# baurst/liso

Measured on AMD Instinct MI355X. Metric: LISO train-step frames/sec (120k-pt clouds), higher is better.
Workload: dtype bf16 (detector, BASELINE configs[2]) + f32 via bf16x3 MFMA (SLIM); north_star's 1e-3 on logits / flow is met by `parity_leg` (f32 via bf16x3 MFMA everywhere) and `fp32_exact_leg`, not by the bf16 detector

## Files before the change

### include/liso_flow_cluster.h

```cpp
#ifndef LISO_FLOW_CLUSTER_H
#define LISO_FLOW_CLUSTER_H

#include <stddef.h>
#include <stdint.h>

#ifdef __cplusplus
extern "C" {
#endif

size_t liso_bev_dynamic_flow_workspace_bytes(int batch, int h, int w);

int liso_bev_dynamic_flow_f32(const float* points, int point_stride, const uint8_t* valid, const int32_t* pillar_coors,
                              const float* flow, int flow_stride, const double* odom_minus_eye, int batch, int n, int h,
                              int w, float* dynamicness, float* nonrigid_flow, void* workspace, size_t workspace_bytes,
                              void* stream);

int liso_odom_inverse_minus_eye_f64(const double* odom, int batch, double* out, void* stream);

size_t liso_fit_box_z_workspace_bytes(int n_points, int n_boxes);

int liso_fit_box_z_f32(const float* points, int point_stride, int n, const float* box_pos, int pos_dims,
                       const float* box_dims, int dims_dims, const float* box_rot, int k, float box_height,
                       int64_t* num_pts, float* fitted_z, float* fitted_height, void* workspace, size_t workspace_bytes,
                       void* stream);

// ... 1 lines not shown
    int batch, gx, gy;
    int window;
    int min_samples;
    float eps;
    float flow_weight;
} liso_dbscan_cfg;

int liso_dbscan_components(const liso_dbscan_cfg* cfg, const uint8_t* dynamic_mask, const float* row_coords,
                           const float* col_coords, const float* flow, uint8_t* core, int32_t* parent, int32_t* is_root,
                           void* stream);

int liso_dbscan_labels(const liso_dbscan_cfg* cfg, const uint8_t* dynamic_mask, const float* row_coords, const float* col_coords,
                       const float* flow, const uint8_t* core, const int32_t* parent, const int32_t* root_rank,
                       int32_t* labels, void* stream);

int liso_region_props(const int32_t* labels, int batch, int gx, int gy, int max_labels, uint64_t* moments, double* props,
                      void* stream);

size_t liso_region_props_workspace_bytes(int batch, int gx, int gy, int max_labels);
int liso_region_props_ws(const int32_t* labels, int batch, int gx, int gy, int max_labels, uint64_t* moments, double* props,
                         void* workspace, size_t workspace_bytes, void* stream);

#ifdef __cplusplus
}
#endif
#endif
```

### liso_amd/_lib.py

```python
import ctypes
import os

import torch

_HERE = os.path.dirname(os.path.abspath(__file__))
LIB_PATH = os.path.join(_HERE, "libliso_hip.so")

_lib = None


class LisoHipError(RuntimeError):
    pass


_ERRORS = {-1: "LISO_EINVAL (bad pointer/size)", -2: "LISO_EWORKSPACE (workspace too small)",
           -3: "LISO_ELAUNCH (HIP launch failed)", -4: "LISO_GROUND_ELENGTH (int(67 / delta_R) > 255)"}


def _preload_torch_hip_runtime():
    tl = os.path.join(os.path.dirname(torch.__file__), "lib", "libamdhip64.so")
    if os.path.exists(tl):
        ctypes.CDLL(tl, mode=ctypes.RTLD_GLOBAL)


# ... 105 lines not shown
    "liso_pfn_forward_rows": (_i, [_vp, _vp, _vp, _vp, _i, _vp, _vp, _vp, _vp, _i, _i, _vp, _vp, _vp]),
    "liso_pfn_backward": (_i, [_vp, _vp, _vp, _vp, _i, _vp, _vp, _vp, _vp, _vp, _i, _vp, _i, _vp, _vp, _vp, _vp, _vp]),
    "liso_pfn_bn_prepare_sub_f32": (_i, [_vp, _vp, _vp, _i, _i, _vp, _vp, _vp, _vp, _vp, _vp, _f, _f, _i, _vp, _vp, _vp, _vp]),
    "liso_pfn_forward_scatter_sub": (_i, [_vp, _vp, _vp, _vp, _i, _i, _vp, _vp, _vp, _vp, _i, _vp, _vp]),
    "liso_pfn_forward_rows_sub": (_i, [_vp, _vp, _vp, _vp, _i, _i, _vp, _vp, _vp, _vp, _i, _i, _vp, _vp, _vp]),
    "liso_pfn_backward_sub": (_i, [_vp, _vp, _vp, _vp, _i, _i, _vp, _vp, _vp, _vp, _vp, _i, _vp, _i, _vp, _vp, _vp, _vp, _vp]),
    "liso_kabsch_workspace_bytes": (_sz, [_vp]),
    "liso_kabsch_trafos_f32": (_i, [_vp, _vp, _vp, _vp, _vp, _vp, _vp, _vp, _vp, _vp, _vp, _sz, _vp]),
    "liso_kabsch_trafos_counted_f32": (_i, [_vp, _vp, _vp, _vp, _vp, _vp, _vp, _vp, _vp, _vp, _vp, _vp, _sz, _vp]),
    "liso_symm_ortho_fwd_f64": (_i, [_vp, _i, _vp, _vp, _vp, _vp, _vp]),
    "liso_symm_ortho_bwd_f64": (_i, [_vp, _vp, _vp, _vp, _i, _vp, _vp]),
    "liso_weighted_moments_workspace_bytes": (_sz, [_i]),
    "liso_weighted_moments_fwd_f32": (_i, [_vp, _vp, _vp, _i, ctypes.c_long, _vp, _vp, _sz, _vp]),
    "liso_weighted_moments_bwd_f32": (_i, [_vp, _vp, _vp, _i, ctypes.c_long, _vp, _vp, _vp, _vp, _vp]),
    "liso_bev_dynamic_flow_workspace_bytes": (_sz, [_i, _i, _i]),
    "liso_bev_dynamic_flow_f32": (_i, [_vp, _i, _vp, _vp, _vp, _i, _vp, _i, _i, _i, _i, _vp, _vp, _vp, _sz, _vp]),
    "liso_odom_inverse_minus_eye_f64": (_i, [_vp, _i, _vp, _vp]),
    "liso_fit_box_z_workspace_bytes": (_sz, [_i, _i]),
    "liso_fit_box_z_f32": (_i, [_vp, _i, _i, _vp, _i, _vp, _i, _vp, _i, _f, _vp, _vp, _vp, _vp, _sz, _vp]),
    "liso_dbscan_components": (_i, [_vp, _vp, _vp, _vp, _vp, _vp, _vp, _vp, _vp]),
    "liso_dbscan_labels": (_i, [_vp, _vp, _vp, _vp, _vp, _vp, _vp, _vp, _vp, _vp]),
    "liso_region_props": (_i, [_vp, _i, _i, _i, _i, _vp, _vp, _vp]),
    "liso_region_props_workspace_bytes": (_sz, [_i, _i, _i, _i]),
    "liso_region_props_ws": (_i, [_vp, _i, _i, _i, _i, _vp, _vp, _vp, _sz, _vp]),
    "liso_corr_lookup_fwd_f32": (_i, [_vp, _vp, _vp, _vp, _vp, _vp]),
    "liso_corr_lookup_fwd_tiled_f32": (_i, [_vp, _vp, _vp, _vp, _vp, _vp]),
    "liso_corr_lookup_bwd_dvol_f32": (_i, [_vp, _vp, _vp, _vp, _vp]),
    "liso_corr_pyramid_fwd_f32": (_i, [_vp, _vp, _vp, _vp]),
    "liso_corr_pyramid_bwd_f32": (_i, [_vp, _vp, _vp, _vp]),
    "liso_corr_bwd_features_workspace_bytes": (_sz, [_vp]),
    "liso_corr_bwd_features_f32": (_i, [_vp, _i, _vp, _vp, _vp, _vp, _vp, _vp, _sz, _vp]),
    "liso_rows_combine_f32": (_i, [_lg, _i, _vp, _lg, _vp, _lg, _vp, _lg, _vp, _lg, _vp, _lg, _i, _vp]),
    "liso_gru_out_rows_train_f32": (_i, [_lg, _i, _vp, _lg, _vp, _vp, _lg, _vp, _lg, _vp]),
    "liso_gru_out_rows_bwd_f32": (_i, [_lg, _i, _vp, _lg, _vp, _vp, _lg, _vp, _lg, _vp, _lg, _vp, _vp, _vp]),
    "liso_gru_in_rows_bwd_f32": (_i, [_lg, _i, _vp, _lg, _vp, _lg, _vp, _vp, _vp, _lg, _vp, _lg, _vp, _vp]),
    "liso_raft_state_step_train_f32": (_i, [_i, _i, _vp, _vp, _vp, _vp, _vp, _vp, _vp, _vp, _vp]),
# ... 392 lines not shown
```

### liso_amd/csrc/flow_cluster.hip

```cpp
#include <hip/hip_runtime.h>
#include "zero_fill.h"
#include <math.h>
#include <stdint.h>

#include "../../include/liso_flow_cluster.h"
#include "../../include/liso_iou3d.h"
#include "dev_common.h"

namespace {

using liso_dev::check_launch;

constexpr double kFix = 16777216.0;

__global__ __launch_bounds__(256) void bev_scatter_kernel(const float* __restrict__ points, int ps, const uint8_t* __restrict__ valid,
                                   const int32_t* __restrict__ coors, const float* __restrict__ flow, int fs,
                                   const double* __restrict__ ome, int batch, int n, int h, int w,
                                   long long* __restrict__ sums, int* __restrict__ counts) {
    const size_t i = (size_t)blockIdx.x * blockDim.x + threadIdx.x;
    const int lane = threadIdx.x & 63;
    long long cell = -1;
    long long q[4] = {0, 0, 0, 0};
    if (i < (size_t)batch * n && valid[i]) {
        const int b = (int)(i / n);
        const int r = coors[i * 2 + 0], c = coors[i * 2 + 1];
        if (r >= 0 && r < h && c >= 0 && c < w) {
            const float* p = points + i * ps;
            const float* f = flow + i * fs;
            const double* M = ome + (size_t)b * 16;
            const double x = p[0], y = p[1], z = p[2];
            float nr[3];
#pragma unroll
            for (int k = 0; k < 3; k++) {
                const float stat = (float)(M[k * 4 + 0] * x + M[k * 4 + 1] * y + M[k * 4 + 2] * z + M[k * 4 + 3]);
                nr[k] = f[k] - stat;
            }
            const float len = sqrtf(nr[0] * nr[0] + nr[1] * nr[1] + nr[2] * nr[2]);
            cell = (long long)(((size_t)b * h + r) * w + c);
            q[0] = llrint((double)len * kFix);
            q[1] = llrint((double)nr[0] * kFix);
            q[2] = llrint((double)nr[1] * kFix);
            q[3] = llrint((double)nr[2] * kFix);
        }
    }
    const long long prev = __shfl_up(cell, 1);
    const bool head = lane == 0 || prev != cell;
    const unsigned long long heads = __ballot(head);
    const int run = __popcll(heads & ((2ull << lane) - 1ull));
    int cnt = cell >= 0 ? 1 : 0;
#pragma unroll
    for (int o = 1; o < 64; o <<= 1) {
        const int other_run = __shfl_down(run, o);
        const bool take = lane + o < 64 && other_run == run;
#pragma unroll
        for (int k = 0; k < 4; k++) {
            const long long v = __shfl_down(q[k], o);
            if (take) q[k] += v;
        }
        const int vc = __shfl_down(cnt, o);
        if (take) cnt += vc;
    }
    if (!head || cell < 0) return;
    unsigned long long* s = (unsigned long long*)(sums + cell * 4);
    atomicAdd(s + 0, (unsigned long long)q[0]);
    atomicAdd(s + 1, (unsigned long long)q[1]);
    atomicAdd(s + 2, (unsigned long long)q[2]);
    atomicAdd(s + 3, (unsigned long long)q[3]);
    atomicAdd(&counts[cell], cnt);
}

__global__ void bev_mean_kernel(const long long* __restrict__ sums, const int* __restrict__ counts, size_t cells,
                                float* __restrict__ dyn, float* __restrict__ nrflow) {
    const size_t i = (size_t)blockIdx.x * blockDim.x + threadIdx.x;
    if (i >= cells) return;
    const int cnt = counts[i];
    float v[4];
#pragma unroll
    for (int k = 0; k < 4; k++) {
        v[k] = (float)((double)sums[i * 4 + k] / kFix);
        if (cnt > 1) v[k] = v[k] / (float)cnt;
    }
    dyn[i] = v[0];
    nrflow[i * 3 + 0] = v[1]; nrflow[i * 3 + 1] = v[2]; nrflow[i * 3 + 2] = v[3];
}

constexpr int kFitThreads = 256;
constexpr int kFitTile = 256;
constexpr int kFitMaxBlocks = 256;

struct FitPartial {
    int count;
    float zmin, zmax, zmin_sensor;
    int zmin_idx;
};
// ... 122 lines not shown

inline int fit_blocks(int n) {
    const int tiles = (n + kFitTile - 1) / kFitTile;
    return tiles < kFitMaxBlocks ? (tiles > 0 ? tiles : 1) : kFitMaxBlocks;
}

}

extern "C" {

size_t liso_bev_dynamic_flow_workspace_bytes(int batch, int h, int w) {
    if (batch <= 0 || h <= 0 || w <= 0) return 0;
    return (size_t)batch * h * w * (4 * sizeof(long long) + sizeof(int));
}

int liso_bev_dynamic_flow_f32(const float* points, int point_stride, const uint8_t* valid, const int32_t* pillar_coors,
                              const float* flow, int flow_stride, const double* odom_minus_eye, int batch, int n, int h,
                              int w, float* dynamicness, float* nonrigid_flow, void* workspace, size_t workspace_bytes,
                              void* stream) {
    if (batch <= 0 || n < 0 || h <= 0 || w <= 0 || point_stride < 3 || flow_stride < 3) return LISO_EINVAL;
    if (!dynamicness || !nonrigid_flow || !workspace || !odom_minus_eye) return LISO_EINVAL;
    if (n > 0 && (!points || !valid || !pillar_coors || !flow)) return LISO_EINVAL;
    const size_t need = liso_bev_dynamic_flow_workspace_bytes(batch, h, w);
    if (workspace_bytes < need) return LISO_EWORKSPACE;
    hipStream_t st = (hipStream_t)stream;
    const size_t cells = (size_t)batch * h * w;
    long long* sums = (long long*)workspace;
    int* counts = (int*)(sums + cells * 4);
    if (liso_zero::zero_async(workspace, need, st) != hipSuccess) return LISO_ELAUNCH;
    const size_t total = (size_t)batch * n;
    if (total > 0)
        bev_scatter_kernel<<<(unsigned)((total + 255) / 256), 256, 0, st>>>(points, point_stride, valid, pillar_coors, flow,
                                                                          flow_stride, odom_minus_eye, batch, n, h, w, sums,
                                                                          counts);
    bev_mean_kernel<<<(unsigned)((cells + 255) / 256), 256, 0, st>>>(sums, counts, cells, dynamicness, nonrigid_flow);
    return check_launch();
}

int liso_odom_inverse_minus_eye_f64(const double* odom, int batch, double* out, void* stream) {
    if (batch < 0 || (batch > 0 && (!odom || !out))) return LISO_EINVAL;
    if (batch == 0) return LISO_OK;
    odom_inverse_minus_eye_kernel<<<(batch + 63) / 64, 64, 0, (hipStream_t)stream>>>(odom, batch, out);
    return check_launch();
}

size_t liso_fit_box_z_workspace_bytes(int n_points, int n_boxes) {
    if (n_points < 0 || n_boxes <= 0) return 0;
    return (size_t)fit_blocks(n_points) * n_boxes * sizeof(FitPartial);
}

// ... 24 lines not shown
```

### liso_amd/csrc/flow_dbscan.hip

```cpp
#include <hip/hip_runtime.h>
#include "zero_fill.h"
#include <math.h>
#include <stdint.h>
#include <stdlib.h>

#include "../../include/liso_flow_cluster.h"
#include "../../include/liso_iou3d.h"
#include "dev_common.h"

namespace {

using liso_dev::check_launch;

struct Cfg {
    int batch, gx, gy, win, min_samples;
    double eps_sqr;
    float flow_weight;
};

__device__ __forceinline__ double dist_sqr(const float* __restrict__ xs, const float* __restrict__ ys,
                                           const float* __restrict__ flow, float fw, int r0, int c0, size_t i0, int r1, int c1,
                                           size_t i1) {
    const double d0 = (double)xs[r0] - (double)xs[r1];
    const double d1 = (double)ys[c0] - (double)ys[c1];
// ... 123 lines not shown
            if (other >= me) return;
            int x = me, y = other;
            while (true) {
                x = find_root_compress(par, x);
                y = find_root_compress(par, y);
                if (x == y) break;
                if (x < y) { const int t = x; x = y; y = t; }
                const int old = atomicMin(&par[x], y);
                if (old == x) break;
                x = old;
            }
        });
    }
}

constexpr int kTR = 16, kTC = 32, kUfThreads = 256, kMaxWin = 8;
constexpr int kRegMax = (kTR + 2 * kMaxWin) * (kTC + 2 * kMaxWin);

__device__ __forceinline__ int lds_find(const int* par, int l, int r0, int c0, int RW, int gy) {
    while (true) {
        const int me = (r0 + l / RW) * gy + (c0 + l % RW);
        const int p = par[l];
        if (p == me) return l;
        l = (p / gy - r0) * RW + (p % gy - c0);
    }
}

__global__ __launch_bounds__(kUfThreads) void dbscan_union_tiled_kernel(Cfg c, const uint8_t* __restrict__ dyn,
                                                                        const uint8_t* __restrict__ core, const float* __restrict__ xs,
                                                                        const float* __restrict__ ys, const float* __restrict__ flow,
                                                                        int* __restrict__ parent, int tiles_r, int tiles_c) {
// ... 119 lines not shown
        const int* par = parent + (size_t)b * per;
        const int* rank = root_rank + (size_t)b * per;
        if (core[i]) {
            label = rank[find_root(par, (int)(i % per))];
        } else {
            int best = 0x7fffffff;
            for_each_neighbour(c, dyn, xs, ys, flow, b, r, col, [&](size_t nb) {
                if (core[nb]) best = min(best, rank[find_root(par, (int)(nb % per))]);
            });
            label = best == 0x7fffffff ? 0 : best;
        }
    }
    labels[i] = label;
}

__global__ __launch_bounds__(256) void region_moments_kernel(const int* __restrict__ labels, int batch, int gx, int gy, int max_labels,
                                                             unsigned long long* __restrict__ mom) {
    const unsigned i = blockIdx.x * blockDim.x + threadIdx.x;
    const unsigned per = (unsigned)gx * (unsigned)gy;
    const int lane = threadIdx.x & 63;
    int l = i < per * (unsigned)batch ? labels[i] : 0;
    if (l > max_labels) l = 0;
    const unsigned bi = i / per, rem = i - bi * per, ri = rem / (unsigned)gy;
    const long key = l > 0 ? (long)bi * max_labels + (l - 1) : -1;
    const unsigned long long r = ri, col = rem - ri * (unsigned)gy;
    unsigned long long todo = __ballot(key >= 0);
    while (todo) {
        const int src = __ffsll((long long)todo) - 1;
        const long k = __shfl(key, src);
        const bool mine = key == k;
// ... 80 lines not shown
    p[0] = cr; p[1] = cc; p[2] = orientation; p[3] = 4.0 * sqrt(l1); p[4] = 4.0 * sqrt(l2);
}

inline bool cfg_ok(const liso_dbscan_cfg* c) {
    return c && c->batch >= 1 && c->gx >= 1 && c->gy >= 1 && c->window >= 0 && c->min_samples >= 1 && c->eps > 0.f &&
           (long)c->gx * c->gy < (1L << 31);
}
inline Cfg to_cfg(const liso_dbscan_cfg* c) {
    Cfg k;
    k.batch = c->batch; k.gx = c->gx; k.gy = c->gy; k.win = c->window; k.min_samples = c->min_samples;
    k.eps_sqr = (double)c->eps * (double)c->eps;
    k.flow_weight = c->flow_weight;
    return k;
}

}

extern "C" {

int liso_dbscan_components(const liso_dbscan_cfg* cfg, const uint8_t* dynamic_mask, const float* row_coords,
                           const float* col_coords, const float* flow, uint8_t* core, int32_t* parent, int32_t* is_root,
                           void* stream) {
    if (!cfg_ok(cfg) || !dynamic_mask || !row_coords || !col_coords || !flow || !core || !parent || !is_root) return LISO_EINVAL;
    const Cfg c = to_cfg(cfg);
    const size_t total = (size_t)c.batch * c.gx * c.gy;
    const unsigned blocks = (unsigned)((total + 255) / 256);
    hipStream_t st = (hipStream_t)stream;
    dbscan_core_kernel<<<blocks, 256, 0, st>>>(c, dynamic_mask, row_coords, col_coords, flow, core, parent);
    if (c.win <= kMaxWin) {
        const int tiles_r = (c.gx + kTR - 1) / kTR, tiles_c = (c.gy + kTC - 1) / kTC;
// ... 6 lines not shown
    return check_launch();
}

int liso_dbscan_labels(const liso_dbscan_cfg* cfg, const uint8_t* dynamic_mask, const float* row_coords, const float* col_coords,
                       const float* flow, const uint8_t* core, const int32_t* parent, const int32_t* root_rank,
                       int32_t* labels, void* stream) {
    if (!cfg_ok(cfg) || !dynamic_mask || !row_coords || !col_coords || !flow || !core || !parent || !root_rank || !labels)
        return LISO_EINVAL;
    const Cfg c = to_cfg(cfg);
    const size_t total = (size_t)c.batch * c.gx * c.gy;
    dbscan_label_kernel<<<(unsigned)((total + 255) / 256), 256, 0, (hipStream_t)stream>>>(c, dynamic_mask, core, row_coords,
                                                                                       col_coords, flow, parent, root_rank, labels);
    return check_launch();
}

int liso_region_props(const int32_t* labels, int batch, int gx, int gy, int max_labels, uint64_t* moments, double* props,
                      void* stream) {
    if (!labels || batch < 1 || gx < 1 || gy < 1 || max_labels < 1 || !moments || !props) return LISO_EINVAL;
    if ((size_t)batch * gx * gy >= (1ull << 31)) return LISO_EINVAL;
    hipStream_t st = (hipStream_t)stream;
    const size_t total = (size_t)batch * gx * gy;
    const long regions = (long)batch * max_labels;
    if (liso_zero::zero_async(moments, (size_t)regions * 6 * sizeof(uint64_t), st) != hipSuccess) return LISO_ELAUNCH;
    region_moments_kernel<<<(unsigned)((total + 255) / 256), 256, 0, st>>>(labels, batch, gx, gy, max_labels,
                                                                          (unsigned long long*)moments);
    region_props_kernel<<<(unsigned)((regions + 255) / 256), 256, 0, st>>>((const unsigned long long*)moments, regions, props);
    return check_launch();
}

size_t liso_region_props_workspace_bytes(int batch, int gx, int gy, int max_labels) {
// ... 26 lines not shown
```

### liso_amd/csrc/kabsch.hip

```cpp
#include <hip/hip_runtime.h>
#include <math.h>
#include <stdint.h>

#include "../../include/liso_iou3d.h"
#include "../../include/liso_kabsch.h"
#include "dev_common.h"

namespace {

using liso_dev::check_launch;

constexpr int kThreads = 256;
constexpr int kTile = 128;
constexpr int kPtsPerWave = kTile / 4;
constexpr int kMaxBlocks = 512;
constexpr int NM = LISO_KABSCH_NMOM;
constexpr float kPi = 3.14159265358979323846f;

struct BoxP {
    float cx, cy, cz, c, s, hl, hw, hh;
};

__device__ __forceinline__ float soft(float x, int softness) {
    return softness == 0 ? 0.5f + (1.0f / kPi) * atanf(x) : 1.0f / (1.0f + expf(-x));
// ... 223 lines not shown
        const double nv = sqrt(v[0] * v[0] + v[1] * v[1] + v[2] * v[2]);
        for (int i = 0; i < 3; i++) o.U[i][1] = v[i] / nv;
        rank = 2;
    }
    if (rank == 2) {
        const double detV = o.V[0][0] * (o.V[1][1] * o.V[2][2] - o.V[1][2] * o.V[2][1]) -
                            o.V[0][1] * (o.V[1][0] * o.V[2][2] - o.V[1][2] * o.V[2][0]) +
                            o.V[0][2] * (o.V[1][0] * o.V[2][1] - o.V[1][1] * o.V[2][0]);
        const double sgn = detV >= 0 ? 1.0 : -1.0;
        o.U[0][2] = sgn * (o.U[1][0] * o.U[2][1] - o.U[2][0] * o.U[1][1]);
        o.U[1][2] = sgn * (o.U[2][0] * o.U[0][1] - o.U[0][0] * o.U[2][1]);
        o.U[2][2] = sgn * (o.U[0][0] * o.U[1][1] - o.U[1][0] * o.U[0][1]);
    }
}

__global__ __launch_bounds__(64) void kabsch_solve_kernel(liso_kabsch_cfg cfg, const float* __restrict__ partials,
                                                          int nblk, const float* __restrict__ box_pos,
                                                          double* __restrict__ trafos, float* __restrict__ cum_wts) {
    const int S = cfg.n_slots;
    const int b = blockIdx.y, slot = blockIdx.x;
    const int lane = threadIdx.x;
    double m[NM], u[NM];
#pragma unroll
    for (int k = 0; k < NM; k++) m[k] = u[k] = 0.0;
    for (int blk = lane; blk < nblk; blk += 64) {
        const float* p = partials + ((size_t)b * nblk + blk) * (S + 2) * NM;
#pragma unroll
        for (int k = 0; k < NM; k++) { m[k] += (double)p[slot * NM + k]; u[k] += (double)p[(S + 1) * NM + k]; }
    }
#pragma unroll
    for (int k = 0; k < NM; k++)
        for (int o = 32; o > 0; o >>= 1) { m[k] += __shfl_xor(m[k], o); u[k] += __shfl_xor(u[k], o); }
    if (lane != 0) return;
    double cx = 0.0, cy = 0.0;
    if (slot < S) { cx = (double)box_pos[((size_t)b * S + slot) * 3 + 0]; cy = (double)box_pos[((size_t)b * S + slot) * 3 + 1]; }
    double W = m[0];
    if ((float)W < 1e-12f) {
        const double eps = (double)1e-12f;
        for (int k = 0; k < NM; k++) m[k] = eps * u[k];
        m[0] = eps * (double)cfg.n_points;
        W = m[0];
        cx = 0.0; cy = 0.0;
    }
    const double mx0 = m[1] / W, mx1 = m[2] / W, my0 = m[3] / W, my1 = m[4] / W;
    double A[3][3] = {{m[5] / W - my0 * mx0, m[6] / W - my0 * mx1, 0.0},
                      {m[7] / W - my1 * mx0, m[8] / W - my1 * mx1, 0.0},
                      {0.0, 0.0, 0.0}};
    Svd3 sv;
    jacobi_svd3(A, sv);
    double R[3][3];
    for (int i = 0; i < 3; i++)
        for (int j = 0; j < 3; j++) R[i][j] = sv.U[i][0] * sv.V[j][0] + sv.U[i][1] * sv.V[j][1] + sv.U[i][2] * sv.V[j][2];
    const double X0 = mx0 + cx, X1 = mx1 + cy, Y0 = my0 + cx, Y1 = my1 + cy;
    double* T = trafos + ((size_t)b * (S + 1) + slot) * 16;
    for (int i = 0; i < 3; i++) {
        for (int j = 0; j < 3; j++) T[i * 4 + j] = R[i][j];
        const double yi = i == 0 ? Y0 : (i == 1 ? Y1 : 0.0);
        T[i * 4 + 3] = yi - (R[i][0] * X0 + R[i][1] * X1);
// ... 118 lines not shown
```

### liso_amd/networks/flow_cluster_detector/flow_cluster_detector.py

```python
import numpy as np
import torch

from liso_amd import _lib as L
from liso_amd.kabsch.shape_utils import Shape, extract_motion_in_pred_box_coordinates
from liso_amd.utils.bev_flow_utils import get_bev_dynamic_flow_map_from_pcl_flow_and_odom


@torch.no_grad()
def fit_bev_box_z_and_height_using_points_in_box(pcl, boxes: Shape, box_height=1000.0):
    assert len(pcl.shape) == 2, pcl.shape
    assert len(boxes.pos.shape) == 2, boxes.pos.shape
    L.require_cuda(pcl)
    dev = pcl.device
    pts = pcl.float().contiguous()
    K = boxes.pos.shape[0]
    num = torch.zeros(K, dtype=torch.int64, device=dev)
    fz = torch.zeros(K, dtype=torch.float32, device=dev)
    fh = torch.zeros(K, dtype=torch.float32, device=dev)
    if K == 0:
        return num, fz, fh
    pos, dims, rot = boxes.pos.float().contiguous(), boxes.dims.float().contiguous(), boxes.rot[..., 0].float().contiguous()
    lib = L.lib()
    nbytes = lib.liso_fit_box_z_workspace_bytes(pts.shape[0], K)
    ws = torch.empty(max(nbytes, 8), dtype=torch.uint8, device=dev)
# ... 11 lines not shown
    B, gx, gy = dynamic_mask.shape
    dev = dynamic_mask.device
    dyn = dynamic_mask.to(torch.uint8).contiguous()
    flow = bev_nonrigid_flow.float().contiguous()
    assert flow.shape == (B, gx, gy, 3), flow.shape
    xs, ys = row_coords_m.float().contiguous(), col_coords_m.float().contiguous()
    if pitch is None:
        pitch = min(float(xs[1] - xs[0]) if gx > 1 else eps, float(ys[1] - ys[0]) if gy > 1 else eps)
    cfg = L.DbscanCfg(B, gx, gy, int(eps / pitch) + 1, int(min_samples), float(eps), float(flow_similarity_importance))
    core = torch.empty((B, gx, gy), dtype=torch.uint8, device=dev)
    parent = torch.empty((B, gx, gy), dtype=torch.int32, device=dev)
    is_root = torch.empty((B, gx, gy), dtype=torch.int32, device=dev)
    labels = torch.empty((B, gx, gy), dtype=torch.int32, device=dev)
    lib = L.lib()
    import ctypes
    with torch.cuda.device(dev):
        L.check(L.TIMER.launch("dbscan_components", lambda: lib.liso_dbscan_components(
            ctypes.byref(cfg), L.ptr(dyn), L.ptr(xs), L.ptr(ys), L.ptr(flow), L.ptr(core), L.ptr(parent), L.ptr(is_root),
            L.stream_ptr())), "dbscan_components")
        from liso_amd.networks.flow_cluster_detector.mining_ops import inclusive_scan_i32
        rank = inclusive_scan_i32(is_root.view(B, -1)).view(B, gx, gy)
        L.check(L.TIMER.launch("dbscan_labels", lambda: lib.liso_dbscan_labels(
            ctypes.byref(cfg), L.ptr(dyn), L.ptr(xs), L.ptr(ys), L.ptr(flow), L.ptr(core), L.ptr(parent), L.ptr(rank),
            L.ptr(labels), L.stream_ptr())), "dbscan_labels")
    return labels, rank.view(B, -1)[:, -1].long()


@torch.no_grad()
def label_region_props(labels, max_labels):
    L.require_cuda(labels)
    B, gx, gy = labels.shape
    lab = labels.to(torch.int32).contiguous()
    mom = torch.empty((B, max_labels, 6), dtype=torch.int64, device=lab.device)
    props = torch.empty((B, max_labels, 5), dtype=torch.float64, device=lab.device)
    lib = L.lib()
    nbytes = lib.liso_region_props_workspace_bytes(B, gx, gy, max_labels)
    ws = torch.empty(max(nbytes, 8), dtype=torch.uint8, device=lab.device)
    with torch.cuda.device(lab.device):
        L.check(L.TIMER.launch("region_props", lambda: lib.liso_region_props_ws(
# ... 111 lines not shown
```

### liso_amd/utils/bev_flow_utils.py

```python
import torch

from liso_amd import _lib as L


@torch.no_grad()
def get_bev_dynamic_flow_map_from_pcl_flow_and_odom(*, pcl_is_valid, pcl, pillar_coors, point_flow, odom_ta_tb,
                                                    target_shape, return_nonrigid_bev_flow=False, odom_minus_eye=None):
    L.require_cuda(pcl, point_flow)
    B, N = pcl_is_valid.shape
    h, w = int(target_shape[0]), int(target_shape[1])
    dev = pcl.device
    pts = pcl.float().contiguous()
    fl = point_flow.float().contiguous()
    assert fl.shape[-1] >= 3, fl.shape
    val = pcl_is_valid.to(torch.uint8).contiguous()
    coors = pillar_coors.to(torch.int32).contiguous()
    ome = odom_minus_eye if odom_minus_eye is not None else odometry_minus_identity(odom_ta_tb)
    dyn = torch.empty((B, h, w, 1), dtype=torch.float32, device=dev)
    nrf = torch.empty((B, h, w, 3), dtype=torch.float32, device=dev)
    lib = L.lib()
    nbytes = lib.liso_bev_dynamic_flow_workspace_bytes(B, h, w)
    ws = torch.empty(nbytes, dtype=torch.uint8, device=dev)
    with torch.cuda.device(dev):
        L.check(L.TIMER.launch("bev_dynamic_flow", lambda: lib.liso_bev_dynamic_flow_f32(
            L.ptr(pts), pts.shape[-1], L.ptr(val), L.ptr(coors), L.ptr(fl), fl.shape[-1], L.ptr(ome), B, N, h, w,
            L.ptr(dyn), L.ptr(nrf), L.ptr(ws), nbytes, L.stream_ptr())), "bev_dynamic_flow")
    if return_nonrigid_bev_flow:
        return dyn, nrf
    return dyn


@torch.no_grad()
def odometry_minus_identity(odom_ta_tb):
    dev = odom_ta_tb.device
    if not odom_ta_tb.is_cuda:
        return (torch.linalg.inv_ex(odom_ta_tb.double()).inverse - torch.eye(4, device=dev, dtype=torch.float64)[None]).contiguous()
# ... 6 lines not shown
```

Baseline: 1061.

## Aggregate BEV scatter in LDS hash, compact DBSCAN active lists, tune Kabsch reduce

The BEV dynamic-flow scatter now processes 1024-point chunks per block. It merges same-cell contributions in a shared-memory hash table before issuing global atomics, and it can use an interleaved 5-word per-cell record layout. DBSCAN gains workspace-based entry points that first compact the dynamic cells into a list via count and scan kernels, so the core and label kernels touch only active cells; the union block size is also raised to 1024. The Kabsch solve unrolls its partials reduction with several rows loaded ahead and reduces the fallback row only when the weight is near zero. The aim is to cut global atomic contention and wasted work on sparse grids, at the cost of extra launches and more shared-memory pressure.

```diff
diff --git a/include/liso_flow_cluster.h b/include/liso_flow_cluster.h
--- a/include/liso_flow_cluster.h
+++ b/include/liso_flow_cluster.h
@@ -9,6 +9,8 @@
 #endif
 
 size_t liso_bev_dynamic_flow_workspace_bytes(int batch, int h, int w);
+
+size_t liso_bev_dynamic_flow_record_workspace_bytes(int batch, int h, int w);
 
 int liso_bev_dynamic_flow_f32(const float* points, int point_stride, const uint8_t* valid, const int32_t* pillar_coors,
                               const float* flow, int flow_stride, const double* odom_minus_eye, int batch, int n, int h,
@@ -40,6 +42,14 @@
                        const float* flow, const uint8_t* core, const int32_t* parent, const int32_t* root_rank,
                        int32_t* labels, void* stream);
 
+size_t liso_dbscan_workspace_bytes(const liso_dbscan_cfg* cfg);
+int liso_dbscan_components_ws(const liso_dbscan_cfg* cfg, const uint8_t* dynamic_mask, const float* row_coords,
+                              const float* col_coords, const float* flow, uint8_t* core, int32_t* parent, int32_t* is_root,
+                              void* workspace, size_t workspace_bytes, void* stream);
+int liso_dbscan_labels_ws(const liso_dbscan_cfg* cfg, const uint8_t* dynamic_mask, const float* row_coords, const float* col_coords,
+                          const float* flow, const uint8_t* core, const int32_t* parent, const int32_t* root_rank, int32_t* labels,
+                          const void* workspace, size_t workspace_bytes, void* stream);
+
 int liso_region_props(const int32_t* labels, int batch, int gx, int gy, int max_labels, uint64_t* moments, double* props,
                       void* stream);
 
diff --git a/liso_amd/_lib.py b/liso_amd/_lib.py
--- a/liso_amd/_lib.py
+++ b/liso_amd/_lib.py
@@ -143,12 +143,16 @@
     "liso_weighted_moments_fwd_f32": (_i, [_vp, _vp, _vp, _i, ctypes.c_long, _vp, _vp, _sz, _vp]),
     "liso_weighted_moments_bwd_f32": (_i, [_vp, _vp, _vp, _i, ctypes.c_long, _vp, _vp, _vp, _vp, _vp]),
     "liso_bev_dynamic_flow_workspace_bytes": (_sz, [_i, _i, _i]),
+    "liso_bev_dynamic_flow_record_workspace_bytes": (_sz, [_i, _i, _i]),
     "liso_bev_dynamic_flow_f32": (_i, [_vp, _i, _vp, _vp, _vp, _i, _vp, _i, _i, _i, _i, _vp, _vp, _vp, _sz, _vp]),
     "liso_odom_inverse_minus_eye_f64": (_i, [_vp, _i, _vp, _vp]),
     "liso_fit_box_z_workspace_bytes": (_sz, [_i, _i]),
     "liso_fit_box_z_f32": (_i, [_vp, _i, _i, _vp, _i, _vp, _i, _vp, _i, _f, _vp, _vp, _vp, _vp, _sz, _vp]),
     "liso_dbscan_components": (_i, [_vp, _vp, _vp, _vp, _vp, _vp, _vp, _vp, _vp]),
     "liso_dbscan_labels": (_i, [_vp, _vp, _vp, _vp, _vp, _vp, _vp, _vp, _vp, _vp]),
+    "liso_dbscan_workspace_bytes": (_sz, [_vp]),
+    "liso_dbscan_components_ws": (_i, [_vp, _vp, _vp, _vp, _vp, _vp, _vp, _vp, _vp, _sz, _vp]),
+    "liso_dbscan_labels_ws": (_i, [_vp, _vp, _vp, _vp, _vp, _vp, _vp, _vp, _vp, _vp, _sz, _vp]),
     "liso_region_props": (_i, [_vp, _i, _i, _i, _i, _vp, _vp, _vp]),
     "liso_region_props_workspace_bytes": (_sz, [_i, _i, _i, _i]),
     "liso_region_props_ws": (_i, [_vp, _i, _i, _i, _i, _vp, _vp, _vp, _sz, _vp]),
diff --git a/liso_amd/csrc/flow_cluster.hip b/liso_amd/csrc/flow_cluster.hip
--- a/liso_amd/csrc/flow_cluster.hip
+++ b/liso_amd/csrc/flow_cluster.hip
@@ -13,71 +13,119 @@
 
 constexpr double kFix = 16777216.0;
 
-__global__ __launch_bounds__(256) void bev_scatter_kernel(const float* __restrict__ points, int ps, const uint8_t* __restrict__ valid,
+template <bool kRecord>
+struct BevAcc {
+    unsigned long long* acc;
+    int* counts;
+    __device__ __forceinline__ unsigned long long* sum(long long cell) const { return acc + cell * (kRecord ? 5 : 4); }
+    __device__ __forceinline__ int* count(long long cell) const { return kRecord ? (int*)(acc + cell * 5 + 4) : counts + cell; }
+    __device__ __forceinline__ void add(long long cell, const long long (&q)[4], int cnt) const {
+        unsigned long long* s = sum(cell);
+        atomicAdd(s + 0, (unsigned long long)q[0]);
+        atomicAdd(s + 1, (unsigned long long)q[1]);
+        atomicAdd(s + 2, (unsigned long long)q[2]);
+        atomicAdd(s + 3, (unsigned long long)q[3]);
+        atomicAdd(count(cell), cnt);
+    }
+};
+
+constexpr int kScThreads = 256, kScChunk = 1024, kScSlotBits = 9, kScSlots = 1 << kScSlotBits, kScProbes = 16;
+constexpr unsigned long long kScEmpty = ~0ull;
+
+template <bool kRecord>
+__global__ __launch_bounds__(kScThreads) void bev_scatter_kernel(const float* __restrict__ points, int ps, const uint8_t* __restrict__ valid,
                                    const int32_t* __restrict__ coors, const float* __restrict__ flow, int fs,
-                                   const double* __restrict__ ome, int batch, int n, int h, int w,
-                                   long long* __restrict__ sums, int* __restrict__ counts) {
-    const size_t i = (size_t)blockIdx.x * blockDim.x + threadIdx.x;
+                                   const double* __restrict__ ome, int batch, int n, int h, int w, BevAcc<kRecord> out) {
+    __shared__ unsigned long long s_key[kScSlots];
+    __shared__ unsigned long long s_sum[kScSlots][4];
+    __shared__ int s_cnt[kScSlots];
+    for (int s = threadIdx.x; s < kScSlots; s += kScThreads) {
+        s_key[s] = kScEmpty;
+        s_sum[s][0] = s_sum[s][1] = s_sum[s][2] = s_sum[s][3] = 0ull;
+        s_cnt[s] = 0;
+    }
+    __syncthreads();
     const int lane = threadIdx.x & 63;
-    long long cell = -1;
-    long long q[4] = {0, 0, 0, 0};
-    if (i < (size_t)batch * n && valid[i]) {
-        const int b = (int)(i / n);
-        const int r = coors[i * 2 + 0], c = coors[i * 2 + 1];
-        if (r >= 0 && r < h && c >= 0 && c < w) {
-            const float* p = points + i * ps;
-            const float* f = flow + i * fs;
-            const double* M = ome + (size_t)b * 16;
-            const double x = p[0], y = p[1], z = p[2];
-            float nr[3];
-#pragma unroll
-            for (int k = 0; k < 3; k++) {
-                const float stat = (float)(M[k * 4 + 0] * x + M[k * 4 + 1] * y + M[k * 4 + 2] * z + M[k * 4 + 3]);
-                nr[k] = f[k] - stat;
-            }
-            const float len = sqrtf(nr[0] * nr[0] + nr[1] * nr[1] + nr[2] * nr[2]);
-            cell = (long long)(((size_t)b * h + r) * w + c);
-            q[0] = llrint((double)len * kFix);
-            q[1] = llrint((double)nr[0] * kFix);
-            q[2] = llrint((double)nr[1] * kFix);
-            q[3] = llrint((double)nr[2] * kFix);
-        }
-    }
-    const long long prev = __shfl_up(cell, 1);
-    const bool head = lane == 0 || prev != cell;
-    const unsigned long long heads = __ballot(head);
-    const int run = __popcll(heads & ((2ull << lane) - 1ull));
-    int cnt = cell >= 0 ? 1 : 0;
-#pragma unroll
-    for (int o = 1; o < 64; o <<= 1) {
-        const int other_run = __shfl_down(run, o);
-        const bool take = lane + o < 64 && other_run == run;
-#pragma unroll
-        for (int k = 0; k < 4; k++) {
-            const long long v = __shfl_down(q[k], o);
-            if (take) q[k] += v;
-        }
-        const int vc = __shfl_down(cnt, o);
-        if (take) cnt += vc;
-    }
-    if (!head || cell < 0) return;
-    unsigned long long* s = (unsigned long long*)(sums + cell * 4);
-    atomicAdd(s + 0, (unsigned long long)q[0]);
-    atomicAdd(s + 1, (unsigned long long)q[1]);
-    atomicAdd(s + 2, (unsigned long long)q[2]);
-    atomicAdd(s + 3, (unsigned long long)q[3]);
-    atomicAdd(&counts[cell], cnt);
-}
-
-__global__ void bev_mean_kernel(const long long* __restrict__ sums, const int* __restrict__ counts, size_t cells,
-                                float* __restrict__ dyn, float* __restrict__ nrflow) {
+    for (int part = 0; part < kScChunk / kScThreads; part++) {
+        const size_t i = (size_t)blockIdx.x * kScChunk + (size_t)part * kScThreads + threadIdx.x;
+        long long cell = -1;
+        long long q[4] = {0, 0, 0, 0};
+        if (i < (size_t)batch * n && valid[i]) {
+            const int b = (int)(i / n);
+            const int r = coors[i * 2 + 0], c = coors[i * 2 + 1];
+            if (r >= 0 && r < h && c >= 0 && c < w) {
+                const float* p = points + i * ps;
+                const float* f = flow + i * fs;
+                const double* M = ome + (size_t)b * 16;
+                const double x = p[0], y = p[1], z = p[2];
+                float nr[3];
+#pragma unroll
+                for (int k = 0; k < 3; k++) {
+                    const float stat = (float)(M[k * 4 + 0] * x + M[k * 4 + 1] * y + M[k * 4 + 2] * z + M[k * 4 + 3]);
+                    nr[k] = f[k] - stat;
+                }
+                const float len = sqrtf(nr[0] * nr[0] + nr[1] * nr[1] + nr[2] * nr[2]);
+                cell = (long long)(((size_t)b * h + r) * w + c);
+                q[0] = llrint((double)len * kFix);
+                q[1] = llrint((double)nr[0] * kFix);
+                q[2] = llrint((double)nr[1] * kFix);
+                q[3] = llrint((double)nr[2] * kFix);
+            }
+        }
+        const long long prev = __shfl_up(cell, 1);
+        const bool head = lane == 0 || prev != cell;
+        const unsigned long long heads = __ballot(head);
+        int cnt = cell >= 0 ? 1 : 0;
+        if (heads != ~0ull) {
+            const int run = __popcll(heads & ((2ull << lane) - 1ull));
+#pragma unroll
+            for (int o = 1; o < 64; o <<= 1) {
+                const int other_run = __shfl_down(run, o);
+                const bool take = lane + o < 64 && other_run == run;
+#pragma unroll
+                for (int k = 0; k < 4; k++) {
+                    const long long v = __shfl_down(q[k], o);
+                    if (take) q[k] += v;
+                }
+                const int vc = __shfl_down(cnt, o);
+                if (take) cnt += vc;
+            }
+        }
+        if (head && cell >= 0) {
+            unsigned s = ((unsigned)cell * 2654435761u) >> (32 - kScSlotBits);
+            bool placed = false;
+            for (int probe = 0; probe < kScProbes; probe++) {
+                const unsigned long long old = atomicCAS(&s_key[s], kScEmpty, (unsigned long long)cell);
+                if (old == kScEmpty || old == (unsigned long long)cell) { placed = true; break; }
+                s = (s + 1) & (kScSlots - 1);
+            }
+            if (placed) {
+#pragma unroll
+                for (int k = 0; k < 4; k++) atomicAdd(&s_sum[s][k], (unsigned long long)q[k]);
+                atomicAdd(&s_cnt[s], cnt);
+            } else {
+                out.add(cell, q, cnt);
+            }
+        }
+    }
+    __syncthreads();
+    for (int s = threadIdx.x; s < kScSlots; s += kScThreads) {
+        if (s_key[s] == kScEmpty) continue;
+        const long long q[4] = {(long long)s_sum[s][0], (long long)s_sum[s][1], (long long)s_sum[s][2], (long long)s_sum[s][3]};
+        out.add((long long)s_key[s], q, s_cnt[s]);
+    }
+}
+
+template <bool kRecord>
+__global__ void bev_mean_kernel(BevAcc<kRecord> in, size_t cells, float* __restrict__ dyn, float* __restrict__ nrflow) {
     const size_t i = (size_t)blockIdx.x * blockDim.x + threadIdx.x;
     if (i >= cells) return;
-    const int cnt = counts[i];
+    const int cnt = *in.count((long long)i);
+    const long long* sums = (const long long*)in.sum((long long)i);
     float v[4];
 #pragma unroll
     for (int k = 0; k < 4; k++) {
-        v[k] = (float)((double)sums[i * 4 + k] / kFix);
+        v[k] = (float)((double)sums[k] / kFix);
         if (cnt > 1) v[k] = v[k] / (float)cnt;
     }
     dyn[i] = v[0];
@@ -230,6 +278,11 @@
     return (size_t)batch * h * w * (4 * sizeof(long long) + sizeof(int));
 }
 
+size_t liso_bev_dynamic_flow_record_workspace_bytes(int batch, int h, int w) {
+    if (batch <= 0 || h <= 0 || w <= 0) return 0;
+    return (size_t)batch * h * w * (5 * sizeof(long long));
+}
+
 int liso_bev_dynamic_flow_f32(const float* points, int point_stride, const uint8_t* valid, const int32_t* pillar_coors,
                               const float* flow, int flow_stride, const double* odom_minus_eye, int batch, int n, int h,
                               int w, float* dynamicness, float* nonrigid_flow, void* workspace, size_t workspace_bytes,
@@ -241,15 +294,25 @@
     if (workspace_bytes < need) return LISO_EWORKSPACE;
     hipStream_t st = (hipStream_t)stream;
     const size_t cells = (size_t)batch * h * w;
-    long long* sums = (long long*)workspace;
-    int* counts = (int*)(sums + cells * 4);
-    if (liso_zero::zero_async(workspace, need, st) != hipSuccess) return LISO_ELAUNCH;
     const size_t total = (size_t)batch * n;
-    if (total > 0)
-        bev_scatter_kernel<<<(unsigned)((total + 255) / 256), 256, 0, st>>>(points, point_stride, valid, pillar_coors, flow,
-                                                                          flow_stride, odom_minus_eye, batch, n, h, w, sums,
-                                                                          counts);
-    bev_mean_kernel<<<(unsigned)((cells + 255) / 256), 256, 0, st>>>(sums, counts, cells, dynamicness, nonrigid_flow);
+    const unsigned chunks = (unsigned)((total + kScChunk - 1) / kScChunk), mean_blocks = (unsigned)((cells + 255) / 256);
+    unsigned long long* acc = (unsigned long long*)workspace;
+    const size_t record_need = liso_bev_dynamic_flow_record_workspace_bytes(batch, h, w);
+    if (workspace_bytes >= record_need) {
+        const BevAcc<true> a{acc, nullptr};
+        if (liso_zero::zero_async(workspace, record_need, st) != hipSuccess) return LISO_ELAUNCH;
+        if (total > 0)
+            bev_scatter_kernel<true><<<chunks, kScThreads, 0, st>>>(points, point_stride, valid, pillar_coors, flow, flow_stride,
+                                                                    odom_minus_eye, batch, n, h, w, a);
+        bev_mean_kernel<true><<<mean_blocks, 256, 0, st>>>(a, cells, dynamicness, nonrigid_flow);
+    } else {
+        const BevAcc<false> a{acc, (int*)(acc + cells * 4)};
+        if (liso_zero::zero_async(workspace, need, st) != hipSuccess) return LISO_ELAUNCH;
+        if (total > 0)
+            bev_scatter_kernel<false><<<chunks, kScThreads, 0, st>>>(points, point_stride, valid, pillar_coors, flow, flow_stride,
+                                                                     odom_minus_eye, batch, n, h, w, a);
+        bev_mean_kernel<false><<<mean_blocks, 256, 0, st>>>(a, cells, dynamicness, nonrigid_flow);
+    }
     return check_launch();
 }
 
diff --git a/liso_amd/csrc/flow_dbscan.hip b/liso_amd/csrc/flow_dbscan.hip
--- a/liso_amd/csrc/flow_dbscan.hip
+++ b/liso_amd/csrc/flow_dbscan.hip
@@ -161,7 +161,7 @@
     }
 }
 
-constexpr int kTR = 16, kTC = 32, kUfThreads = 256, kMaxWin = 8;
+constexpr int kTR = 16, kTC = 32, kUfThreads = 1024, kMaxWin = 8;
 constexpr int kRegMax = (kTR + 2 * kMaxWin) * (kTC + 2 * kMaxWin);
 
 __device__ __forceinline__ int lds_find(const int* par, int l, int r0, int c0, int RW, int gy) {
@@ -311,6 +311,105 @@
     labels[i] = label;
 }
 
+constexpr int kListThreads = 256, kListPasses = 8, kListTile = kListThreads * kListPasses;
+constexpr int kListGrid = 1024;
+
+__global__ __launch_bounds__(kListThreads) void dyn_count_kernel(const uint8_t* __restrict__ dyn, unsigned total, int* __restrict__ block_cnt) {
+    __shared__ int wsum[kListThreads / 64];
+    const unsigned base = blockIdx.x * (unsigned)kListTile;
+    int n = 0;
+#pragma unroll
+    for (int k = 0; k < kListPasses; k++) {
+        const unsigned i = base + k * kListThreads + threadIdx.x;
+        n += (i < total && dyn[i]) ? 1 : 0;
+    }
+#pragma unroll
+    for (int o = 32; o > 0; o >>= 1) n += __shfl_xor(n, o);
+    if ((threadIdx.x & 63) == 0) wsum[threadIdx.x >> 6] = n;
+    __syncthreads();
+    if (threadIdx.x == 0) block_cnt[blockIdx.x] = (wsum[0] + wsum[1]) + (wsum[2] + wsum[3]);
+}
+
+__global__ __launch_bounds__(kListThreads) void dyn_list_kernel(const uint8_t* __restrict__ dyn, unsigned total, const int* __restrict__ block_cnt,
+                                                                int* __restrict__ list, int* __restrict__ n_list, uint8_t* __restrict__ core,
+                                                                int* __restrict__ parent) {
+    __shared__ int s_red[kListThreads / 64];
+    __shared__ int s_seg[kListPasses][kListThreads / 64];
+    const int lane = threadIdx.x & 63, wave = threadIdx.x >> 6;
+    int before = 0;
+    for (int q = threadIdx.x; q < (int)blockIdx.x; q += kListThreads) before += block_cnt[q];
+#pragma unroll
+    for (int o = 32; o > 0; o >>= 1) before += __shfl_xor(before, o);
+    if (lane == 0) s_red[wave] = before;
+    const unsigned base = blockIdx.x * (unsigned)kListTile;
+    unsigned long long mine[kListPasses];
+#pragma unroll
+    for (int k = 0; k < kListPasses; k++) {
+        const unsigned i = base + k * kListThreads + threadIdx.x;
+        const bool d = i < total && dyn[i];
+        mine[k] = __ballot(d);
+        if (lane == 0) s_seg[k][wave] = __popcll(mine[k]);
+        if (i < total && !d) { core[i] = 0; parent[i] = -1; }
+    }
+    __syncthreads();
+    int pos = (s_red[0] + s_red[1]) + (s_red[2] + s_red[3]);
+#pragma unroll
+    for (int k = 0; k < kListPasses; k++) {
+        if ((mine[k] >> lane) & 1ull) {
+            int p = pos + __popcll(mine[k] & ((1ull << lane) - 1ull));
+            for (int w = 0; w < wave; w++) p += s_seg[k][w];
+            list[p] = (int)(base + k * kListThreads + threadIdx.x);
+        }
+        pos += (s_seg[k][0] + s_seg[k][1]) + (s_seg[k][2] + s_seg[k][3]);
+    }
+    if (blockIdx.x == gridDim.x - 1 && threadIdx.x == 0) *n_list = pos;
+}
+
+__global__ __launch_bounds__(256) void dbscan_core_list_kernel(Cfg c, const uint8_t* __restrict__ dyn, const float* __restrict__ xs,
+                                                               const float* __restrict__ ys, const float* __restrict__ flow,
+                                                               const int* __restrict__ list, const int* __restrict__ n_list,
+                                                               uint8_t* __restrict__ core, int* __restrict__ parent) {
+    const int lane = threadIdx.x & 63, n = *n_list;
+    const size_t per = (size_t)c.gx * c.gy;
+    for (int e = blockIdx.x * 4 + (threadIdx.x >> 6); e < n; e += gridDim.x * 4) {
+        const size_t cell = (size_t)list[e];
+        int count = 0;
+        wave_for_each_neighbour(c, dyn, xs, ys, flow, cell, lane, [&](size_t) { count++; });
+#pragma unroll
+        for (int o = 32; o > 0; o >>= 1) count += __shfl_xor(count, o);
+        if (lane == 0) {
+            const int is_core = count >= c.min_samples;
+            core[cell] = (uint8_t)is_core;
+            parent[cell] = is_core ? (int)(cell % per) : -1;
+        }
+    }
+}
+
+__global__ __launch_bounds__(256) void dbscan_label_list_kernel(Cfg c, const uint8_t* __restrict__ dyn, const uint8_t* __restrict__ core,
+                                                                const float* __restrict__ xs, const float* __restrict__ ys,
+                                                                const float* __restrict__ flow, const int* __restrict__ parent,
+                                                                const int* __restrict__ root_rank, const int* __restrict__ list,
+                                                                const int* __restrict__ n_list, int* __restrict__ labels) {
+    const int lane = threadIdx.x & 63, n = *n_list;
+    const size_t per = (size_t)c.gx * c.gy;
+    for (int e = blockIdx.x * 4 + (threadIdx.x >> 6); e < n; e += gridDim.x * 4) {
+        const size_t cell = (size_t)list[e];
+        const int* par = parent + (cell / per) * per;
+        const int* rank = root_rank + (cell / per) * per;
+        int best = 0x7fffffff;
+        if (core[cell]) {
+            best = rank[find_root(par, (int)(cell % per))];
+        } else {
+            wave_for_each_neighbour(c, dyn, xs, ys, flow, cell, lane, [&](size_t nb) {
+                if (core[nb]) best = min(best, rank[find_root(par, (int)(nb % per))]);
+            });
+#pragma unroll
+            for (int o = 32; o > 0; o >>= 1) best = min(best, __shfl_xor(best, o));
+        }
+        if (lane == 0) labels[cell] = best == 0x7fffffff ? 0 : best;
+    }
+}
+
 __global__ __launch_bounds__(256) void region_moments_kernel(const int* __restrict__ labels, int batch, int gx, int gy, int max_labels,
                                                              unsigned long long* __restrict__ mom) {
     const unsigned i = blockIdx.x * blockDim.x + threadIdx.x;
@@ -421,6 +520,20 @@
     return k;
 }
 
+struct ListWs {
+    int *list, *block_cnt, *n_list;
+    unsigned blocks;
+};
+inline size_t carve_list(void* base, size_t total, ListWs& w) {
+    liso_dev::Carver cv{base};
+    w.blocks = (unsigned)((total + kListTile - 1) / kListTile);
+    w.list = cv.take<int>(total);
+    w.block_cnt = cv.take<int>(w.blocks);
+    w.n_list = cv.take<int>(1);
+    return cv.bytes;
+}
+inline unsigned list_grid(size_t total) { return (unsigned)(total / 4 + 1 < (size_t)kListGrid ? total / 4 + 1 : (size_t)kListGrid); }
+
 }
 
 extern "C" {
@@ -457,6 +570,58 @@
     return check_launch();
 }
 
+size_t liso_dbscan_workspace_bytes(const liso_dbscan_cfg* cfg) {
+    if (!cfg_ok(cfg) || (size_t)cfg->batch * cfg->gx * cfg->gy >= (1ull << 31)) return 0;
+    ListWs w{};
+    return carve_list(nullptr, (size_t)cfg->batch * cfg->gx * cfg->gy, w);
+}
+
+int liso_dbscan_components_ws(const liso_dbscan_cfg* cfg, const uint8_t* dynamic_mask, const float* row_coords,
+                              const float* col_coords, const float* flow, uint8_t* core, int32_t* parent, int32_t* is_root,
+                              void* workspace, size_t workspace_bytes, void* stream) {
+    if (!cfg_ok(cfg) || !dynamic_mask || !row_coords || !col_coords || !flow || !core || !parent || !is_root) return LISO_EINVAL;
+    const size_t need = liso_dbscan_workspace_bytes(cfg);
+    if (need == 0) return LISO_EINVAL;
+    if (!workspace || workspace_bytes < need) return LISO_EWORKSPACE;
+    const Cfg c = to_cfg(cfg);
+    const size_t total = (size_t)c.batch * c.gx * c.gy;
+    ListWs w{};
+    carve_list(workspace, total, w);
+    hipStream_t st = (hipStream_t)stream;
+    dyn_count_kernel<<<w.blocks, kListThreads, 0, st>>>(dynamic_mask, (unsigned)total, w.block_cnt);
+    dyn_list_kernel<<<w.blocks, kListThreads, 0, st>>>(dynamic_mask, (unsigned)total, w.block_cnt, w.list, w.n_list, core, parent);
+    dbscan_core_list_kernel<<<list_grid(total), 256, 0, st>>>(c, dynamic_mask, row_coords, col_coords, flow, w.list, w.n_list, core,
+                                                             parent);
+    if (c.win <= kMaxWin) {
+        const int tiles_r = (c.gx + kTR - 1) / kTR, tiles_c = (c.gy + kTC - 1) / kTC;
+        dbscan_union_tiled_kernel<<<dim3(tiles_r * tiles_c, c.batch), kUfThreads, 0, st>>>(c, dynamic_mask, core, row_coords, col_coords,
+                                                                                         flow, parent, tiles_r, tiles_c);
+    } else {
+        dbscan_union_kernel<<<(unsigned)((total + 255) / 256), 256, 0, st>>>(c, dynamic_mask, core, row_coords, col_coords, flow, parent);
+    }
+    dbscan_flatten_kernel<<<(unsigned)((total + 255) / 256), 256, 0, st>>>(c, core, parent, is_root);
+    return check_launch();
+}
+
+int liso_dbscan_labels_ws(const liso_dbscan_cfg* cfg, const uint8_t* dynamic_mask, const float* row_coords, const float* col_coords,
+                          const float* flow, const uint8_t* core, const int32_t* parent, const int32_t* root_rank, int32_t* labels,
+                          const void* workspace, size_t workspace_bytes, void* stream) {
+    if (!cfg_ok(cfg) || !dynamic_mask || !row_coords || !col_coords || !flow || !core || !parent || !root_rank || !labels)
+        return LISO_EINVAL;
+    const size_t need = liso_dbscan_workspace_bytes(cfg);
+    if (need == 0) return LISO_EINVAL;
+    if (!workspace || workspace_bytes < need) return LISO_EWORKSPACE;
+    const Cfg c = to_cfg(cfg);
+    const size_t total = (size_t)c.batch * c.gx * c.gy;
+    ListWs w{};
+    carve_list((void*)workspace, total, w);
+    hipStream_t st = (hipStream_t)stream;
+    if (liso_zero::zero_async(labels, total * sizeof(int32_t), st) != hipSuccess) return LISO_ELAUNCH;
+    dbscan_label_list_kernel<<<list_grid(total), 256, 0, st>>>(c, dynamic_mask, core, row_coords, col_coords, flow, parent, root_rank,
+                                                              w.list, w.n_list, labels);
+    return check_launch();
+}
+
 int liso_region_props(const int32_t* labels, int batch, int gx, int gy, int max_labels, uint64_t* moments, double* props,
                       void* stream) {
     if (!labels || batch < 1 || gx < 1 || gy < 1 || max_labels < 1 || !moments || !props) return LISO_EINVAL;
diff --git a/liso_amd/csrc/kabsch.hip b/liso_amd/csrc/kabsch.hip
--- a/liso_amd/csrc/kabsch.hip
+++ b/liso_amd/csrc/kabsch.hip
@@ -261,34 +261,55 @@
     }
 }
 
+constexpr int kRowsAhead = 8;
+__device__ __forceinline__ void reduce_rows(const float* __restrict__ partials, int b, int nblk, int S, int row, int lane,
+                                            double (&m)[NM]) {
+#pragma unroll
+    for (int k = 0; k < NM; k++) m[k] = 0.0;
+    for (int blk0 = lane; blk0 < nblk; blk0 += 64 * kRowsAhead) {
+        float v[kRowsAhead][NM];
+#pragma unroll
+        for (int j = 0; j < kRowsAhead; j++) {
+            const int blk = blk0 + 64 * j;
+            if (blk < nblk) {
+                const float* p = partials + (((size_t)b * nblk + blk) * (S + 2) + row) * NM;
+#pragma unroll
+                for (int k = 0; k < NM; k++) v[j][k] = p[k];
+            }
+        }
+#pragma unroll
+        for (int j = 0; j < kRowsAhead; j++)
+            if (blk0 + 64 * j < nblk) {
+#pragma unroll
+                for (int k = 0; k < NM; k++) m[k] += (double)v[j][k];
+            }
+    }
+#pragma unroll
+    for (int k = 0; k < NM; k++)
+        for (int o = 32; o > 0; o >>= 1) m[k] += __shfl_xor(m[k], o);
+}
+
 __global__ __launch_bounds__(64) void kabsch_solve_kernel(liso_kabsch_cfg cfg, const float* __restrict__ partials,
                                                           int nblk, const float* __restrict__ box_pos,
                                                           double* __restrict__ trafos, float* __restrict__ cum_wts) {
     const int S = cfg.n_slots;
     const int b = blockIdx.y, slot = blockIdx.x;
     const int lane = threadIdx.x;
-    double m[NM], u[NM];
-#pragma unroll
-    for (int k = 0; k < NM; k++) m[k] = u[k] = 0.0;
-    for (int blk = lane; blk < nblk; blk += 64) {
-        const float* p = partials + ((size_t)b * nblk + blk) * (S + 2) * NM;
-#pragma unroll
-        for (int k = 0; k < NM; k++) { m[k] += (double)p[slot * NM + k]; u[k] += (double)p[(S + 1) * NM + k]; }
-    }
-#pragma unroll
-    for (int k = 0; k < NM; k++)
-        for (int o = 32; o > 0; o >>= 1) { m[k] += __shfl_xor(m[k], o); u[k] += __shfl_xor(u[k], o); }
-    if (lane != 0) return;
+    double m[NM];
+    reduce_rows(partials, b, nblk, S, slot, lane, m);
     double cx = 0.0, cy = 0.0;
     if (slot < S) { cx = (double)box_pos[((size_t)b * S + slot) * 3 + 0]; cy = (double)box_pos[((size_t)b * S + slot) * 3 + 1]; }
     double W = m[0];
     if ((float)W < 1e-12f) {
+        double u[NM];
+        reduce_rows(partials, b, nblk, S, S + 1, lane, u);
         const double eps = (double)1e-12f;
         for (int k = 0; k < NM; k++) m[k] = eps * u[k];
         m[0] = eps * (double)cfg.n_points;
         W = m[0];
         cx = 0.0; cy = 0.0;
     }
+    if (lane != 0) return;
     const double mx0 = m[1] / W, mx1 = m[2] / W, my0 = m[3] / W, my1 = m[4] / W;
     double A[3][3] = {{m[5] / W - my0 * mx0, m[6] / W - my0 * mx1, 0.0},
                       {m[7] / W - my1 * mx0, m[8] / W - my1 * mx1, 0.0},
diff --git a/liso_amd/networks/flow_cluster_detector/flow_cluster_detector.py b/liso_amd/networks/flow_cluster_detector/flow_cluster_detector.py
--- a/liso_amd/networks/flow_cluster_detector/flow_cluster_detector.py
+++ b/liso_amd/networks/flow_cluster_detector/flow_cluster_detector.py
@@ -49,15 +49,17 @@
     labels = torch.empty((B, gx, gy), dtype=torch.int32, device=dev)
     lib = L.lib()
     import ctypes
+    nbytes = lib.liso_dbscan_workspace_bytes(ctypes.byref(cfg))
+    ws = torch.empty(max(nbytes, 8), dtype=torch.uint8, device=dev)
     with torch.cuda.device(dev):
-        L.check(L.TIMER.launch("dbscan_components", lambda: lib.liso_dbscan_components(
-            ctypes.byref(cfg), L.ptr(dyn), L.ptr(xs), L.ptr(ys), L.ptr(flow), L.ptr(core), L.ptr(parent), L.ptr(is_root),
-            L.stream_ptr())), "dbscan_components")
+        args = (ctypes.byref(cfg), L.ptr(dyn), L.ptr(xs), L.ptr(ys), L.ptr(flow), L.ptr(core), L.ptr(parent), L.ptr(is_root))
+        L.check(L.TIMER.launch("dbscan_components", lambda: lib.liso_dbscan_components_ws(*args, L.ptr(ws), nbytes, L.stream_ptr())
+                               if nbytes else lib.liso_dbscan_components(*args, L.stream_ptr())), "dbscan_components")
         from liso_amd.networks.flow_cluster_detector.mining_ops import inclusive_scan_i32
         rank = inclusive_scan_i32(is_root.view(B, -1)).view(B, gx, gy)
-        L.check(L.TIMER.launch("dbscan_labels", lambda: lib.liso_dbscan_labels(
-            ctypes.byref(cfg), L.ptr(dyn), L.ptr(xs), L.ptr(ys), L.ptr(flow), L.ptr(core), L.ptr(parent), L.ptr(rank),
-            L.ptr(labels), L.stream_ptr())), "dbscan_labels")
+        largs = (ctypes.byref(cfg), L.ptr(dyn), L.ptr(xs), L.ptr(ys), L.ptr(flow), L.ptr(core), L.ptr(parent), L.ptr(rank), L.ptr(labels))
+        L.check(L.TIMER.launch("dbscan_labels", lambda: lib.liso_dbscan_labels_ws(*largs, L.ptr(ws), nbytes, L.stream_ptr())
+                               if nbytes else lib.liso_dbscan_labels(*largs, L.stream_ptr())), "dbscan_labels")
     return labels, rank.view(B, -1)[:, -1].long()
 
 
diff --git a/liso_amd/utils/bev_flow_utils.py b/liso_amd/utils/bev_flow_utils.py
--- a/liso_amd/utils/bev_flow_utils.py
+++ b/liso_amd/utils/bev_flow_utils.py
@@ -19,7 +19,7 @@
     dyn = torch.empty((B, h, w, 1), dtype=torch.float32, device=dev)
     nrf = torch.empty((B, h, w, 3), dtype=torch.float32, device=dev)
     lib = L.lib()
-    nbytes = lib.liso_bev_dynamic_flow_workspace_bytes(B, h, w)
+    nbytes = lib.liso_bev_dynamic_flow_record_workspace_bytes(B, h, w)
     ws = torch.empty(nbytes, dtype=torch.uint8, device=dev)
     with torch.cuda.device(dev):
         L.check(L.TIMER.launch("bev_dynamic_flow", lambda: lib.liso_bev_dynamic_flow_f32(
```

Measured after the change: 1079, median of 6. 1.02x the previous value.
